# reesque/SfmFromScratch

Measured on AMD Instinct MI355X. Metric: images/sec detect+describe+match, 1080p, 1/2/4/8 MI355X, higher is better.
Workload: dtype f32; 1 GPU; BASELINE configs[1]: 32x 1080p per GPU, ScaleRotInvSIFT 4-level x2 octave pyramid, k=2500, fw 18, NNRatio 0.85 over consecutive pairs; frames_per_gpu=32, pairs_per_gpu=31, distinct_batches=2, parallelism=image-shard x1, batches_in_flight=2

## Files before the change

sfmfromscratch_amd/csrc/describe.hip:

```cpp
#include "kernels.h"

#include <stdlib.h>

namespace sfm {

SFM_DEV double pi_edge(int i, int num) {
  const double start = -3.141592653589793, stop = 3.141592653589793;
  if (i == num - 1) return stop;
  double step = (stop - start) / (double)(num - 1);
  return (double)i * step + start;
}

struct DescLayout {
  int ws, n, n4, pw, P;
  size_t off_keys, off_patch, off_ori, off_mag, off_sw, off_cw, off_cellw, off_wgh, total;
};

__host__ __device__ inline DescLayout desc_layout(int fw, int rotate) {
  DescLayout L;
  int h = fw / 2;
  L.ws = 2 * h;
  L.n = L.ws * L.ws;
  L.pw = L.ws + 2;
  int P = 1;
// ... 178 lines not shown
      for (int k = p; k >= 1; k >>= 1)
#pragma unroll
        for (int j = k % p; j + k < 16; j += 2 * k)
#pragma unroll
          for (int i = 0; i < k; ++i) {
            const int a = i + j, c = i + j + k;
            if (c < 16 && a / (2 * p) == c / (2 * p)) {
              const bool sw = cv[a] > cv[c] || (cv[a] == cv[c] && sl[a] > sl[c]);
              const double tv = cv[a];
              cv[a] = sw ? cv[c] : tv;
              cv[c] = sw ? tv : cv[c];
              const float tw = wt[a];
              wt[a] = sw ? wt[c] : tw;
              wt[c] = sw ? tw : wt[c];
              const int ts = sl[a];
              sl[a] = sw ? sl[c] : ts;
              sl[c] = sw ? ts : sl[c];
            }
          }
    float* cw = s_cellw + lane * 17;
    float acc = 0.0f;
    cw[0] = 0.0f;
#pragma unroll
    for (int m = 0; m < 16; ++m) {
      acc = acc + wt[m];
      cw[m + 1] = acc;
    }
    int idx[9];
#pragma unroll
    for (int eb = 0; eb < 9; ++eb) {
      const double e = pi_edge(eb, 9);
      int c = 0;
#pragma unroll
      for (int m = 0; m < 16; ++m) c += (eb < 8) ? (cv[m] < e ? 1 : 0) : (cv[m] <= e ? 1 : 0);
      idx[eb] = c;
    }
#pragma unroll
    for (int bb = 0; bb < 8; ++bb) s_wgh[lane * 8 + bb] = cw[idx[bb + 1]] - cw[idx[bb]];
  }
  __syncthreads();

  float w0 = s_wgh[lane], w1 = s_wgh[lane + 64];
  float a = w0 * w0;
  float c = w1 * w1;
  float s = a + c;
  for (int off = 32; off >= 1; off >>= 1) {
    float o = __shfl_down(s, off);
    s = s + o;
  }
  float nrm = sqrtf(__shfl(s, 0));
  int64_t off0 = 0;
  for (int l = 0; l < level; ++l) off0 += lc_all[(int64_t)l * B + b];
  const int64_t slot = (int64_t)b * out_cap + off0 + kpi;
  float v0 = w0, v1 = w1;
  if (nrm > 0.0f) {
    v0 = v0 / nrm;
    v1 = v1 / nrm;
  }
  out_desc[slot * 128 + lane] = sqrtf(v0);
  out_desc[slot * 128 + lane + 64] = sqrtf(v1);
  if (lane == 0) {
    if (out_conf) out_conf[slot] = kp.conf[ko];
    out_xy[slot * 2 + 0] = (int32_t)((double)x * scale);
    out_xy[slot * 2 + 1] = (int32_t)((double)y * scale);
  }
}

__global__ void k_finalize_counts(const int32_t* __restrict__ lc_all, int B, int L,
                                  int32_t* __restrict__ out_count) {
  int b = blockIdx.x * blockDim.x + threadIdx.x;
  if (b >= B) return;
  int32_t s = 0;
  for (int l = 0; l < L; ++l) s += lc_all[(int64_t)l * B + b];
  out_count[b] = s;
}

size_t describe_lds_bytes(int fw, int rotate) { return desc_layout(fw, rotate).total; }

void init_describe_attributes(size_t max_lds) {
  (void)hipFuncSetAttribute((const void*)k_describe, hipFuncAttributeMaxDynamicSharedMemorySize,
                            (int)max_lds);
}

bool launch_describe(const float* lvl, int B, int H, int W, int fw, int rotate, KpList kp,
                     int kcap, const int32_t* level_counts_all, int level, int L, double scale,
                     int32_t* out_xy, float* out_desc, float* out_conf, int64_t out_cap,
                     int32_t* out_count, const MatchOperands& mo, bool* operands_written, hipStream_t st) {
  if (operands_written) *operands_written = false;
  if (kcap <= 0) return false;
  static const bool one_per_wave = [] {
    const char* v = getenv("SFMFEAT_DESCRIBE");
    return v && v[0] == 'w';
  }();
  if (!one_per_wave && launch_describe_quad(lvl, B, H, W, fw, rotate, kp, kcap, level_counts_all, level,
                                            scale, out_xy, out_desc, out_conf, out_cap, out_count, L, mo, st)) {
    if (operands_written) *operands_written = mo.hi != nullptr;
    return out_count != nullptr;
  }
  size_t lds = describe_lds_bytes(fw, rotate);
  hipLaunchKernelGGL(k_describe, dim3(kcap, B), dim3(64), lds, st, lvl, H, W, fw, rotate, kp, kcap,
                     level_counts_all, level, B, scale, out_xy, out_desc, out_conf, out_cap);
  return false;
}

void launch_finalize_counts(const int32_t* level_counts_all, int B, int L, int32_t* out_count,
                            hipStream_t st) {
  hipLaunchKernelGGL(k_finalize_counts, dim3((B + 255) / 256), dim3(256), 0, st, level_counts_all, B, L,
                     out_count);
}

}
```

sfmfromscratch_amd/csrc/describe_q.hip:

```cpp
#include "kernels.h"

#include <stdlib.h>
#include <string.h>

#include <mutex>

namespace sfm {
namespace dq {

constexpr int cmax(int a, int b) { return a > b ? a : b; }
constexpr int pow2ceil(int v) { return v <= 1 ? 1 : 2 * pow2ceil((v + 1) / 2); }

template <int WS, int ROT>
struct Geo {
  static constexpr int N = WS * WS, PW = WS + 2, NP = PW * PW;
  static constexpr int P = cmax(pow2ceil(N), 16), E = P / 16;
  static constexpr int RN = (N + 15) / 16;
  static constexpr int A = (cmax(cmax(NP, N + 4), 16 * 17) + 3) & ~3;
  static constexpr int NQ = (N + 3) & ~3;
  static constexpr int OFF_M = A;
  static constexpr int OFF_K = OFF_M + NQ;
  static constexpr int OFF_R = OFF_K + NQ;
  static constexpr int OFF_I = OFF_R + (ROT ? (NQ / 2 + 3) & ~3 : 0);
  static constexpr int OFF_T = OFF_I + (ROT ? 40 : 0);
  static constexpr int G = OFF_T + 12;
};

SFM_DEV double pi_edge(int i, int num) {
  const double start = -3.141592653589793, stop = 3.141592653589793;
  if (i == num - 1) return stop;
  const double step = (stop - start) / (double)(num - 1);
  return (double)i * step + start;
}

SFM_DEV uint32_t edge_key(double e, double sh, bool strict) {
  uint32_t kc = fkey((float)(e + sh));
  auto pass = [&](uint32_t kk) {
    const double d = (double)fkey_inv(kk) - sh;
    return strict ? d > e : d >= e;
  };
  for (int it = 0; it < 64 && pass(kc); ++it) --kc;
  for (int it = 0; it < 64 && !pass(kc); ++it) ++kc;
  return kc;
}

__constant__ uint32_t c_ori[37];
__constant__ uint32_t c_cell[37][9];

template <int CTRL>
SFM_DEV uint32_t dpp(uint32_t v) {
  return (uint32_t)__builtin_amdgcn_update_dpp(0, (int)v, CTRL, 0xF, 0xF, true);
}
template <int X>
SFM_DEV uint32_t rxor(uint32_t v) {
  if constexpr (X == 1) return dpp<0xB1>(v);
  else if constexpr (X == 2) return dpp<0x4E>(v);
  else if constexpr (X == 3) return dpp<0x1B>(v);
  else if constexpr (X == 4) return dpp<0x1B>(dpp<0x141>(v));
  else if constexpr (X == 7) return dpp<0x141>(v);
  else if constexpr (X == 8) return dpp<0x128>(v);
  else {
    static_assert(X == 15, "row-local xor");
    return dpp<0x140>(v);
  }
}
template <int X>
SFM_DEV float rxorf(float v) { return __uint_as_float(rxor<X>(__float_as_uint(v))); }
template <int X>
SFM_DEV double rxord(double v) {
  const uint64_t u = __double_as_longlong(v);
  return __longlong_as_double((long long)(((uint64_t)rxor<X>((uint32_t)(u >> 32)) << 32) | rxor<X>((uint32_t)u)));
}

constexpr uint64_t kBias = 1ull << 52;
constexpr uint64_t kPad = kBias + (1ull << 41);
SFM_DEV double dkey(uint64_t payload) { return __longlong_as_double((long long)(kBias + payload)); }
SFM_DEV uint64_t dpayload(double k) { return (uint64_t)__double_as_longlong(k) - kBias; }

SFM_DEV void cas_up(double& a, double& b) {
  const double lo = __builtin_fmin(a, b), hi = __builtin_fmax(a, b);
  a = lo;
  b = hi;
}
SFM_DEV double keep_or_take(bool lower, double mine, double other) {
  const double lo = __builtin_fmin(mine, other), hi = __builtin_fmax(mine, other);
  return lower ? lo : hi;
}

template <int E, int S>
SFM_DEV void half_clean(double (&k)[E], int gl) {
  if constexpr (S >= 1) {
    if constexpr (S < E) {
#pragma unroll
      for (int r = 0; r < E; ++r)
        if ((r & S) == 0) cas_up(k[r], k[r + S]);
    } else {
      constexpr int X = S / E;
      const bool lower = (gl & X) == 0;
#pragma unroll
      for (int r = 0; r < E; ++r) k[r] = keep_or_take(lower, k[r], rxord<X>(k[r]));
    }
    half_clean<E, S / 2>(k, gl);
  }
}
template <int E, int SIZE>
SFM_DEV void merge_level(double (&k)[E], int gl) {
  if constexpr (SIZE <= 16 * E) {
    if constexpr (SIZE <= E) {
#pragma unroll
      for (int r = 0; r < E; ++r)
        if ((r & (SIZE / 2)) == 0) cas_up(k[r], k[r ^ (SIZE - 1)]);
    } else {
      constexpr int X = SIZE / E - 1;
      const bool lower = (gl & ((X + 1) >> 1)) == 0;
      if constexpr (E == 1) {
        k[0] = keep_or_take(lower, k[0], rxord<X>(k[0]));
      } else {
#pragma unroll
        for (int r = 0; r < E / 2; ++r) {
          const double oa = rxord<X>(k[E - 1 - r]);
          const double ob = rxord<X>(k[r]);
          k[r] = keep_or_take(lower, k[r], oa);
          k[E - 1 - r] = keep_or_take(lower, k[E - 1 - r], ob);
        }
      }
    }
    half_clean<E, SIZE / 4>(k, gl);
    merge_level<E, SIZE * 2>(k, gl);
  }
}

SFM_DEV void grad_at(const float* c, int pw, float& mag, float& ori) {
  const float a00 = c[-pw - 1], a01 = c[-pw], a02 = c[-pw + 1];
  const float a10 = c[-1], a12 = c[1];
  const float a20 = c[pw - 1], a21 = c[pw], a22 = c[pw + 1];
  float gx = 0.0f;
  gx = __builtin_fmaf(-1.0f, a00, gx);
  gx = __builtin_fmaf(1.0f, a02, gx);
  gx = __builtin_fmaf(-2.0f, a10, gx);
  gx = __builtin_fmaf(2.0f, a12, gx);
  gx = __builtin_fmaf(-1.0f, a20, gx);
  gx = __builtin_fmaf(1.0f, a22, gx);
  float gy = 0.0f;
  gy = __builtin_fmaf(-1.0f, a00, gy);
  gy = __builtin_fmaf(-2.0f, a01, gy);
  gy = __builtin_fmaf(-1.0f, a02, gy);
  gy = __builtin_fmaf(1.0f, a20, gy);
  gy = __builtin_fmaf(2.0f, a21, gy);
  gy = __builtin_fmaf(1.0f, a22, gy);
  const float sx = gx * gx;
  const float sy = gy * gy;
  const float s = sx + sy;
  mag = sqrtf(s);
  ori = svml_atan2f(gy, gx);
}

SFM_DEV void cas_up(uint32_t& a, uint32_t& b) {
  const uint32_t lo = min(a, b), hi = max(a, b);
  a = lo;
  b = hi;
}

template <typename T>
SFM_DEV void batcher16(T (&q)[16]) {
#pragma unroll
  for (int p = 1; p < 16; p <<= 1)
#pragma unroll
    for (int kk = p; kk >= 1; kk >>= 1)
#pragma unroll
      for (int j = kk % p; j + kk < 16; j += 2 * kk)
#pragma unroll
        for (int i = 0; i < kk; ++i) {
          const int a = i + j, c = i + j + kk;
          if (c < 16 && a / (2 * p) == c / (2 * p)) cas_up(q[a], q[c]);
        }
}

template <int WS, int ROT, int ABL = 0>
__global__ void __launch_bounds__(64) k_describe_q(const float* __restrict__ lvl, int H, int W, KpList kp,
                                                   int kcap, const int32_t* __restrict__ lc_all, int level,
                                                   int B, double scale, int32_t* __restrict__ out_xy,
                                                   float* __restrict__ out_desc, float* __restrict__ out_conf,
                                                   int64_t out_cap, int32_t* __restrict__ out_count, int L,
                                                   MatchOperands mo) {
  using C = Geo<WS, ROT>;
  constexpr int N = C::N, PW = C::PW, NP = C::NP, E = C::E, RN = C::RN, h = WS / 2;
  __shared__ __attribute__((aligned(16))) float s_all[4 * C::G];
  const int b = blockIdx.y;
  if (out_count != nullptr && blockIdx.x == 0 && threadIdx.x == 0) {
    int32_t s = 0;
    for (int l = 0; l < L; ++l) s += lc_all[(int64_t)l * B + b];
    out_count[b] = s;
  }
  const int nkb = (kcap + 3) / 4;
  if ((int)blockIdx.x >= nkb) {
    int32_t s = 0;
    for (int l = 0; l < L; ++l) s += lc_all[(int64_t)l * B + b];
    const int nt = ((int)gridDim.x - nkb) * 64;
    for (int64_t r = s + ((int)blockIdx.x - nkb) * 64 + threadIdx.x; r < mo.capP; r += nt) {
      const int64_t mr = (int64_t)b * mo.capP + r;
      uint4* hz = reinterpret_cast<uint4*>(mo.hi + mr * 128);
      uint4* lz = reinterpret_cast<uint4*>(mo.lo + mr * 128);
#pragma unroll
      for (int q = 0; q < 16; ++q) {
        hz[q] = make_uint4(0u, 0u, 0u, 0u);
        lz[q] = make_uint4(0u, 0u, 0u, 0u);
      }
      mo.norm2[mr] = INFINITY;
      mo.rnorm[mr] = 0.0f;
    }
    return;
  }
  const int count = kp.count[b];
  const int kbase = blockIdx.x * 4;
  if (kbase >= count) return;
  const int lane = threadIdx.x, g = lane >> 4, gl = lane & 15;
  const int kpi = kbase + g;
  const bool valid = kpi < count;
  const int64_t ko = (int64_t)b * kcap + (valid ? kpi : kbase);
  const int x = kp.x[ko], y = kp.y[ko];
  float* sA = s_all + g * C::G;
  float* sM = sA + C::OFF_M;
  uint32_t* sK = reinterpret_cast<uint32_t*>(sA + C::OFF_K);
  uint16_t* sR = reinterpret_cast<uint16_t*>(sA + C::OFF_R);
  int32_t* sI = reinterpret_cast<int32_t*>(sA + C::OFF_I);
  uint32_t* sT = reinterpret_cast<uint32_t*>(sA + C::OFF_T);

  const float* img = lvl + (int64_t)b * H * W;
#pragma unroll
  for (int it = 0; it < (NP + 15) / 16; ++it) {
    const int e0 = it * 16 + gl;
    const int e = e0 < NP ? e0 : NP - 1;
    const int pr = e / PW, pc = e - pr * PW;
    const int gy = y - h + pr, gx = x - h + pc;
    const bool in = gy >= 0 && gy < H && gx >= 0 && gx < W;
    const int cy = min(max(gy, 0), H - 1), cx = min(max(gx, 0), W - 1);
    const float v = (ABL & 64) ? (float)(cy + cx) : img[(int64_t)cy * W + cx];
    if (e0 < NP) sA[e] = in ? v : 0.0f;
  }
  __syncthreads();

  double k[E];
  bool tiny = false;
#pragma unroll
  for (int r = 0; r < E; ++r) k[r] = __longlong_as_double((long long)kPad);
#pragma unroll
  for (int r = 0; r < RN; ++r) {
    const int e0 = r * 16 + gl;
    const bool ok = (N % 16 == 0) || e0 < N;
    const int e = ok ? e0 : N - 1;
    const int i = e / WS, j = e - i * WS;
    float mag, ori;
    if constexpr ((ABL & 8) != 0) {
      mag = sA[(i + 1) * PW + (j + 1)];
      ori = sA[(i + 1) * PW + j] - 100.0f;
    } else {
      grad_at(sA + (i + 1) * PW + (j + 1), PW, mag, ori);
    }
    if (ok) {
      sM[e] = mag;
// ... 84 lines not shown
    }
    __syncthreads();
    float hb = -INFINITY;
    int bi = 64;
#pragma unroll
    for (int t = 0; t < 3; ++t) {
      const int j = gl + 16 * t;
      if (j < 36) {
        const float v = sA[3 + sI[j + 1]] - sA[3 + sI[j]];
        if (v > hb) { hb = v; bi = j; }
      }
    }
    {
      float ov; int oi;
      ov = rxorf<8>(hb); oi = (int)rxor<8>((uint32_t)bi);
      if (ov > hb || (ov == hb && oi < bi)) { hb = ov; bi = oi; }
      ov = rxorf<4>(hb); oi = (int)rxor<4>((uint32_t)bi);
      if (ov > hb || (ov == hb && oi < bi)) { hb = ov; bi = oi; }
      ov = rxorf<2>(hb); oi = (int)rxor<2>((uint32_t)bi);
      if (ov > hb || (ov == hb && oi < bi)) { hb = ov; bi = oi; }
      ov = rxorf<1>(hb); oi = (int)rxor<1>((uint32_t)bi);
      if (ov > hb || (ov == hb && oi < bi)) { hb = ov; bi = oi; }
    }
    dom = (pi_edge(bi, 37) + pi_edge(bi + 1, 37)) / 2.0;
    dom_bin = bi;
  }

  if (gl < 9) sT[gl] = (ABL & 32) ? 0x80000000u + (uint32_t)(dom * 1e6) * gl : c_cell[dom_bin][gl];
  __syncthreads();
  float hv[8];
  if constexpr ((ABL & 4) != 0) {
#pragma unroll
    for (int bb = 0; bb < 8; ++bb) hv[bb] = sM[gl * 8 + bb] + __uint_as_float(sT[bb & 7]);
  } else {
  const int r4 = gl >> 2, c4 = gl & 3;
  float wv[16];
  uint32_t hk[16];
  const bool grp_tiny = ROT && ((__ballot(tiny) >> (16 * g)) & 0xFFFFull) != 0;
  if (ROT && !grp_tiny) {
    uint32_t q[16];
#pragma unroll
    for (int t = 0; t < 16; ++t) {
      const int i = 4 * r4 + (t >> 2), j = 4 * c4 + (t & 3);
      const bool ok = i < WS && j < WS;
      q[t] = ok ? (uint32_t)sR[ok ? i * WS + j : 0] : 0xFFFFFFFFu;
    }
    batcher16(q);
#pragma unroll
    for (int m = 0; m < 16; ++m) {
      const bool ok = q[m] != 0xFFFFFFFFu;
      const uint32_t p = ok ? q[m] : 0u;
      wv[m] = ok ? sM[p] : 0.0f;
      hk[m] = ok ? sK[p] : 0xFFFFFFFFu;
    }
  } else {
    uint64_t q[16];
#pragma unroll
    for (int t = 0; t < 16; ++t) {
      const int i = 4 * r4 + (t >> 2), j = 4 * c4 + (t & 3);
      const bool ok = i < WS && j < WS;
      const int e = ok ? i * WS + j : 0;
      const uint32_t key = ROT ? sK[sR[e]] : fkey(__uint_as_float(sK[e]));
      q[t] = ok ? (((uint64_t)key << 32) | (uint32_t)t) : ~0ull;
    }
    if (!ROT) {
      double dq16[16];
#pragma unroll
      for (int t = 0; t < 16; ++t) dq16[t] = q[t] == ~0ull ? __longlong_as_double((long long)kPad)
                                                           : dkey(((q[t] >> 32) << 4) | (uint32_t)t);
      batcher16(dq16);
#pragma unroll
      for (int t = 0; t < 16; ++t) {
        const uint64_t pl = dpayload(dq16[t]);
        q[t] = pl >= (1ull << 36) ? ~0ull : (((pl >> 4) << 32) | (pl & 15u));
      }
    } else {
      double cv[16];
      int sl[16];
#pragma unroll
      for (int t = 0; t < 16; ++t) {
        cv[t] = q[t] == ~0ull ? INFINITY : (double)fkey_inv((uint32_t)(q[t] >> 32)) - dom;
        sl[t] = t;
      }
#pragma unroll
      for (int p = 1; p < 16; p <<= 1)
#pragma unroll
        for (int kk = p; kk >= 1; kk >>= 1)
#pragma unroll
          for (int j = kk % p; j + kk < 16; j += 2 * kk)
#pragma unroll
            for (int i = 0; i < kk; ++i) {
              const int a = i + j, c = i + j + kk;
              if (c < 16 && a / (2 * p) == c / (2 * p)) {
                const bool sw = cv[a] > cv[c] || (cv[a] == cv[c] && sl[a] > sl[c]);
                const double tv = cv[a];
                cv[a] = sw ? cv[c] : tv;
                cv[c] = sw ? tv : cv[c];
                const uint64_t tq = q[a];
                q[a] = sw ? q[c] : tq;
                q[c] = sw ? tq : q[c];
                const int ts = sl[a];
                sl[a] = sw ? sl[c] : ts;
                sl[c] = sw ? ts : sl[c];
              }
            }
    }
#pragma unroll
    for (int m = 0; m < 16; ++m) {
      const bool ok = q[m] != ~0ull;
      const int t = ok ? (int)(uint32_t)q[m] : 0;
      const int e = (4 * r4 + (t >> 2)) * WS + 4 * c4 + (t & 3);
      wv[m] = ok ? (ROT ? sM[sR[e]] : sM[e]) : 0.0f;
      hk[m] = ok ? (uint32_t)(q[m] >> 32) : 0xFFFFFFFFu;
    }
  }
  float* cc = sA + gl * 17;
  float acc = 0.0f;
  cc[0] = 0.0f;
#pragma unroll
  for (int m = 0; m < 16; ++m) {
    acc = acc + wv[m];
    cc[m + 1] = acc;
  }
  int bidx[9];
#pragma unroll
  for (int eb = 0; eb < 9; ++eb) {
    const uint32_t T = sT[eb];
    int c = 0;
#pragma unroll
    for (int m = 0; m < 16; ++m) c += hk[m] < T ? 1 : 0;
    bidx[eb] = c;
  }
#pragma unroll
  for (int bb = 0; bb < 8; ++bb) hv[bb] = cc[bidx[bb + 1]] - cc[bidx[bb]];

  }
  float tr[8];
#pragma unroll
  for (int t = 0; t < 8; ++t) {
    const float a = hv[t] * hv[t];
    tr[t] = a + rxorf<8>(a);
  }
#pragma unroll
  for (int t = 0; t < 8; ++t) tr[t] = tr[t] + rxorf<4>(tr[t]);
#pragma unroll
  for (int t = 0; t < 8; ++t) tr[t] = tr[t] + rxorf<2>(tr[t]);
#pragma unroll
  for (int t = 0; t < 8; ++t) tr[t] = tr[t] + rxorf<1>(tr[t]);
#pragma unroll
  for (int t = 0; t < 4; ++t) tr[t] = tr[t] + tr[t + 4];
  tr[0] = tr[0] + tr[2];
  tr[1] = tr[1] + tr[3];
  tr[0] = tr[0] + tr[1];
  const float nrm = sqrtf(__shfl(tr[0], g * 16));
  if (!valid) return;
  int64_t off0 = 0;
  for (int l = 0; l < level; ++l) off0 += lc_all[(int64_t)l * B + b];
  const int64_t slot = (int64_t)b * out_cap + off0 + kpi;
  float o[8];
#pragma unroll
  for (int t = 0; t < 8; ++t) o[t] = sqrtf(nrm > 0.0f ? hv[t] / nrm : hv[t]);
  float4* dst = reinterpret_cast<float4*>(out_desc + slot * 128 + gl * 8);
  dst[0] = make_float4(o[0], o[1], o[2], o[3]);
  dst[1] = make_float4(o[4], o[5], o[6], o[7]);
  if (mo.hi != nullptr) {
    const int64_t r = off0 + kpi, mr = (int64_t)b * mo.capP + r;
    typedef _Float16 h8 __attribute__((ext_vector_type(8)));
    h8 hh, ll;
    double s = 0.0;
#pragma unroll
    for (int t = 0; t < 8; ++t) {
      const float xs = o[t] * kMatchScale;
      const _Float16 hv16 = (_Float16)xs;
      const float rr = (xs - (float)hv16) * kMatchLoScale;
      hh[t] = hv16;
      ll[t] = (_Float16)rr;
      s += (double)o[t] * (double)o[t];
    }
    *reinterpret_cast<h8*>(mo.hi + mr * 128 + gl * 8) = hh;
    *reinterpret_cast<h8*>(mo.lo + mr * 128 + gl * 8) = ll;
    s += rxord<8>(s);
    s += rxord<4>(s);
    s += rxord<2>(s);
    s += rxord<1>(s);
    if (gl == 0) {
      const float n2 = (float)s, rn = (float)sqrt(s);
      mo.norm2[mr] = n2;
      mo.rnorm[mr] = rn;
      float2* pm = mo.pmax + (int64_t)b * (mo.capP / kPrepRows) + r / kPrepRows;
      atomicMax(reinterpret_cast<unsigned int*>(&pm->x), __float_as_uint(n2));
      atomicMax(reinterpret_cast<unsigned int*>(&pm->y), __float_as_uint(rn));
    }
  }
  if (gl == 0) {
    if (out_conf) out_conf[slot] = kp.conf[ko];
    out_xy[slot * 2 + 0] = (int32_t)((double)x * scale);
    out_xy[slot * 2 + 1] = (int32_t)((double)y * scale);
  }
}

}

namespace {
uint32_t fkey_h(float v) {
  uint32_t b;
  memcpy(&b, &v, 4);
  if (b == 0x80000000u) b = 0u;
  return (b & 0x80000000u) ? ~b : (b | 0x80000000u);
}
float fkey_inv_h(uint32_t k) {
  const uint32_t b = (k & 0x80000000u) ? (k & 0x7fffffffu) : ~k;
  float f;
  memcpy(&f, &b, 4);
  return f;
}
double pi_edge_h(int i, int num) {
  const double start = -3.141592653589793, stop = 3.141592653589793;
  if (i == num - 1) return stop;
  const double step = (stop - start) / (double)(num - 1);
  return (double)i * step + start;
}
uint32_t edge_key_h(double e, double sh, bool strict) {
  uint32_t kc = fkey_h((float)(e + sh));
  auto pass = [&](uint32_t kk) {
    const double d = (double)fkey_inv_h(kk) - sh;
    return strict ? d > e : d >= e;
  };
  for (int it = 0; it < 64 && pass(kc); ++it) --kc;
  for (int it = 0; it < 64 && !pass(kc); ++it) ++kc;
  return kc;
}
}

void init_describe_quad_tables() {
  static std::mutex mu;
  static bool done[256] = {};
  int dev = 0;
  if (hipGetDevice(&dev) != hipSuccess || dev < 0 || dev >= 256) return;
  std::lock_guard<std::mutex> lk(mu);
  if (done[dev]) return;
  uint32_t ori[37], cell[37][9];
  for (int j = 0; j < 37; ++j) ori[j] = edge_key_h(pi_edge_h(j, 37), 0.0, j == 36);
  for (int bi = 0; bi < 37; ++bi) {
    const double dom = bi < 36 ? (pi_edge_h(bi, 37) + pi_edge_h(bi + 1, 37)) / 2.0 : 0.0;
    for (int t = 0; t < 9; ++t) cell[bi][t] = edge_key_h(pi_edge_h(t, 9), dom, t == 8);
  }
  done[dev] = hipMemcpyToSymbol(HIP_SYMBOL(dq::c_ori), ori, sizeof(ori)) == hipSuccess &&
              hipMemcpyToSymbol(HIP_SYMBOL(dq::c_cell), cell, sizeof(cell)) == hipSuccess;
}

#define SFM_DQ_BODY(WS)                                                                              \
    if (rotate)                                                                                      \
      hipLaunchKernelGGL((dq::k_describe_q<WS, 1>), grid, dim3(64), 0, st, lvl, H, W, kp, kcap, lc,  \
                         level, B, scale, out_xy, out_desc, out_conf, out_cap, out_count, L, mo);        \
    else                                                                                             \
      hipLaunchKernelGGL((dq::k_describe_q<WS, 0>), grid, dim3(64), 0, st, lvl, H, W, kp, kcap, lc,  \
                         level, B, scale, out_xy, out_desc, out_conf, out_cap, out_count, L, mo);        \
    return true;
#define SFM_DQ_CASE(WS) \
  case WS:              \
    SFM_DQ_BODY(WS)

bool launch_describe_quad(const float* lvl, int B, int H, int W, int fw, int rotate, KpList kp, int kcap,
                          const int32_t* lc, int level, double scale, int32_t* out_xy, float* out_desc,
                          float* out_conf, int64_t out_cap, int32_t* out_count, int L, const MatchOperands& mo,
                          hipStream_t st) {
  constexpr int kPadBlocks = 8;
  const dim3 grid((kcap + 3) / 4 + (mo.hi != nullptr && out_count != nullptr ? kPadBlocks : 0), B);
  switch (2 * (fw / 2)) {
    SFM_DQ_CASE(2)
    SFM_DQ_CASE(4)
    SFM_DQ_CASE(6)
    SFM_DQ_CASE(8)
    SFM_DQ_CASE(10)
    SFM_DQ_CASE(12)
    SFM_DQ_CASE(14)
    SFM_DQ_CASE(16)
    case 18:
#ifdef SFM_ABLATIONS
      if (rotate) {
        static const int abl = [] {
          const char* v = SFM_ABLATION_ENV("SFMFEAT_DQ_ABL");
          return v ? atoi(v) : 0;
        }();
        switch (abl) {
#define SFM_DQ_ABL(A)                                                                                     \
  case A:                                                                                                \
    hipLaunchKernelGGL((dq::k_describe_q<18, 1, A>), grid, dim3(64), 0, st, lvl, H, W, kp, kcap, lc, level, \
                       B, scale, out_xy, out_desc, out_conf, out_cap, out_count, L, mo);                     \
    return true;
          SFM_DQ_ABL(1)
          SFM_DQ_ABL(2)
          SFM_DQ_ABL(4)
          SFM_DQ_ABL(8)
          SFM_DQ_ABL(7)
          SFM_DQ_ABL(16)
          SFM_DQ_ABL(32)
          SFM_DQ_ABL(64)
          SFM_DQ_ABL(55)
          SFM_DQ_ABL(127)
          default:
            break;
        }
      }
#endif
      SFM_DQ_BODY(18)
    SFM_DQ_CASE(20)
    SFM_DQ_CASE(22)
    default:
      return false;
  }
}

}
```

sfmfromscratch_amd/csrc/kernels.h:

```cpp
#pragma once

#include <hip/hip_runtime.h>
#include <stdint.h>

#include <vector>

#include "common.h"

namespace sfm {

#define SFM_NMS_MAX_HALF 15

constexpr int kHistBits = 12;
constexpr int kHistBins = 1 << kHistBits;
constexpr int kMedBits1 = 11;
constexpr int kMedBins1 = 1 << kMedBits1;
constexpr int kTopkLdsCap = 8192;
constexpr int kMaxMatchRows = 16384;
constexpr int kMatchCandCap = 256;
constexpr int kCounterStride = 32;
constexpr int kMatchUnitPairBits = 20;

constexpr float kMatchScale = 256.0f;
constexpr float kMatchLoScale = 2048.0f;
// ... 131 lines not shown

void ransac_sample_indices(int n, int iters, uint32_t seed, int32_t* out);
void launch_ransac(const int32_t* pts, const int32_t* npts, int nmax, int P, const int32_t* idx,
                   const int32_t* idx_off, int iters, double thr, double* Fs, int32_t* counts, int32_t* out_pts,
                   int32_t* out_n, int32_t* out_iter, hipStream_t st);

int build_resample_table(int in, int out, std::vector<int32_t>& tab);
bool ingest_rows_tables(const std::vector<int32_t>& tab_h, int ks_h, int W, int W2, int ks,
                        std::vector<int32_t>& colmap, std::vector<int32_t>& sets);
int ingest_rows_ks(int ks_h, int ks_v);
void launch_ingest_rgb(const uint8_t* rgb, uint8_t* tmp, float* gray, const int32_t* tab_h, int ks_h,
                       const int32_t* tab_v, int ks_v, const int32_t* colmap, const int32_t* sets, int nsets,
                       int B, int H, int W, int H2, int W2, hipStream_t st);
bool launch_down2x3(const float* src, int sh, int sw, float* d1, float* d2, float* d3, int B, hipStream_t st,
                    void* z0 = nullptr, size_t z0_bytes = 0, void* z1 = nullptr, size_t z1_bytes = 0);
void launch_resize(const float* src, int sh, int sw, float* dst, int dh, int dw, int B,
                   hipStream_t st);

void launch_harris(const float* lvl, float* R, uint32_t* hist, int B, int H, int W,
                   const float* d_gauss, int ks, float alpha, SelectScan scan, hipStream_t st);
constexpr int kHarrisMaxLevels = 4;
struct HarrisLevels {
  struct Level {
    const float* lvl;
    float* R;
    uint32_t* hist;
    int H, W, tiles_x, ntiles, wg0, nwg;
    SelectScan scan;
    float* down[3];
  } l[kHarrisMaxLevels];
  int n;
  int prio;
  int stagger;
  unsigned long long* span;
};
void launch_harris_levels(const HarrisLevels& g, int B, const float* d_gauss, int ks, float alpha,
                          hipStream_t st);
constexpr int kHarrisPairOff = 256;
size_t harris_taps_floats(int ks);
void harris_taps_build(const float* g, int ks, float* out);

int64_t match_stamps_copy(uint64_t* out, int64_t cap);
size_t match_units_words(int P, int max_rows);
float time_harris_ablation(int abl, const float* lvl, float* R, uint32_t* hist, int B, int H, int W,
                           const float* gk, float alpha, int iters, uint64_t* stamps = nullptr,
                           int64_t stamps_cap = 0);

void launch_select_scan(const uint32_t* hist, MedianState* state, unsigned long long* list_count, int B,
                        int H, int W, int64_t vmin, int force_exact, hipStream_t st);
void launch_median_exact(const float* R, MedianState* state, uint32_t* list, unsigned long long* list_count,
                         int B, int H, int W, hipStream_t st);

void launch_nms(const float* R, const MedianState* state, uint64_t* cand,
                unsigned long long* cand_count, int B, int H, int W, int ksize, int mode, hipStream_t st,
                int force_tile = 0);

void init_topk_attributes();
void init_describe_attributes(size_t max_lds);
void init_describe_quad_tables();
size_t describe_lds_bytes(int fw, int rotate);
void launch_select(const float* R, uint64_t* cand, const unsigned long long* cand_count, uint32_t* medlist,
                   uint64_t* scratch, KpList kp, int kcap, int k, int B, int H, int W, int ksize, int half_window,
                   MedianState* state, hipStream_t st);
constexpr int kSelectMaxLevels = 4;
struct SelectLevels {
  struct Level {
    const float* R;
    uint64_t* cand;
    const unsigned long long* cand_count;
    uint32_t* medlist;
    uint64_t* scratch;
    KpList kp;
    MedianState* state;
    int H, W, hw;
  } l[kSelectMaxLevels];
  int n;
};
void launch_select_levels(const SelectLevels& g, int kcap, int k, int B, int ksize, hipStream_t st);

bool launch_describe_quad(const float* lvl, int B, int H, int W, int fw, int rotate, KpList kp, int kcap,
                          const int32_t* level_counts_all, int level, double scale, int32_t* out_xy,
                          float* out_desc, float* out_conf, int64_t out_cap, int32_t* out_count, int L,
                          const MatchOperands& mo, hipStream_t st);
bool launch_describe(const float* lvl, int B, int H, int W, int fw, int rotate, KpList kp,
                     int kcap, const int32_t* level_counts_all, int level, int L, double scale,
                     int32_t* out_xy, float* out_desc, float* out_conf, int64_t out_cap,
                     int32_t* out_count, const MatchOperands& mo, bool* operands_written, hipStream_t st);
void launch_finalize_counts(const int32_t* level_counts_all, int B, int L, int32_t* out_count,
                            hipStream_t st);

struct RowBest {
  int32_t col;
  float nndr;
};
void launch_transpose_desc(const float* desc, const int32_t* count, int nimg, int64_t cap,
                           int64_t capP, float* descT, hipStream_t st);
void launch_match_rows(const float* descT, const int32_t* count, int64_t capP, const int32_t* pairs,
                       int P, float ratio, RowBest* rows, int max_rows, hipStream_t st);
void launch_match_compact(const RowBest* rows, const int32_t* count, const int32_t* pairs, int P,
                          int max_rows, int64_t cap, int32_t* matches, float* conf, int32_t* nmatch,
                          int* reset_counter, hipStream_t st);
void init_match_attributes(int max_rows);
size_t match_pmax_bytes(int64_t capP);
void launch_match_prep(const float* desc, const int32_t* count, int nimg, int64_t cap, int64_t capP,
                       _Float16* hi, _Float16* lo, float* norm2, float* rnorm, void* pmax, hipStream_t st);
void launch_match_mfma(const float* desc, const int32_t* count, int64_t cap, int64_t capP,
                       const _Float16* hi, const _Float16* lo, const float* norm2, const float* rnorm,
                       const void* pmax, const int32_t* pairs, int P, float ratio,
                       RowBest* rows, int max_rows, uint32_t* cand, int32_t* cand_n, float* cand_thr,
                       int* ovf_count, int2* ovf_list, int32_t* units, hipStream_t st);

}
```

sfmfromscratch_amd/csrc/sfmfeat_api.hip:

```cpp
#include <math.h>
#include <stdio.h>
#include <stdlib.h>
#include <string.h>

#include <algorithm>
#include <atomic>
#include <string>
#include <thread>
#include <vector>

#include "../../include/sfmfeat.h"
#include "kernels.h"

using namespace sfm;

namespace {

struct DevBuf {
  void* p = nullptr;
  size_t bytes = 0;
};

struct Level {
  int h, w, fw;
// ... 395 lines not shown
    return SFM_OK;
  };
  for (int l0 = 0; l0 < L;) {
    int l1 = l0 + 1;
    if (group_from > 0 && l0 >= group_from) l1 = std::min(L, l0 + kHarrisMaxLevels);
    {
      StageScope sc(c, SFM_PROF_HARRIS, st);
      HarrisLevels g{};
      g.n = l1 - l0;
      for (int l = l0; l < l1; ++l) {
        const LevelBufs& e = lb[l];
        HarrisLevels::Level& q = g.l[l - l0];
        q.lvl = lvl[l];
        q.R = e.R;
        q.hist = as<uint32_t>(c->d_hist) + (size_t)l * B * kMedBins1;
        q.H = lv[l].h;
        q.W = lv[l].w;
        q.scan = SelectScan{e.med, medcnt + e.co, donecnt + e.co, vmin, e.exact ? 1 : 0};
        q.down[0] = q.down[1] = q.down[2] = nullptr;
        if (pyr_fused && l == 0) {
          q.down[0] = const_cast<float*>(lvl[1]);
          q.down[1] = const_cast<float*>(lvl[2]);
          q.down[2] = const_cast<float*>(lvl[3]);
        }
      }
      if (c->span_cap > 0) {
        if (c->span_n < c->span_cap) {
          g.span = as<unsigned long long>(c->d_spans) + 2 * c->span_n++;
          c->span_level.push_back(l0);
        } else {
          ++c->span_dropped;
        }
      }
      if (!(l0 > 0 && (skip & 16))) launch_harris_levels(g, B, as<float>(c->d_gauss), c->p.gaussian_size, alpha, st);
    }
    if (pyr_fused && l0 == 0 && L > 4) {
      StageScope sc(c, SFM_PROF_PYRAMID, st);
      pyramid_from(4);
    }
    if (gate_level >= l0 && gate_level < l1 && (rc = release_gate())) return rc;
    for (int l = l0; l < l1; ++l) {
      const LevelBufs& e = lb[l];
      if (!e.exact) {
        StageScope sc(c, SFM_PROF_NMS, st);
        launch_nms(e.R, e.med, e.cand, candcnt + e.co, B, lv[l].h, lv[l].w, c->p.ksize, 0, st);
      }
      if (l < L_aux) {
        static const bool sel_caller = [] {
          const char* e = SFM_DIAG_ENV("SFMFEAT_SELECT_CALLER");
          return e && atoi(e) == 1;
        }();
        if (sel_caller) select_level(l, st);
        HIPCHK(c, hipEventRecord(c->ev[l], st));
        HIPCHK(c, hipStreamWaitEvent(ax, c->ev[l], 0));
        if (!sel_caller) select_level(l, ax);
        if (l == L_aux - 1) HIPCHK(c, hipEventRecord(c->ev[L + 2], ax));
        describe_level(l, ax);
      }
    }
    l0 = l1;
  }
  if ((rc = release_gate())) return rc;
  static const bool merge_select = [] {
    const char* e = SFM_DIAG_ENV("SFMFEAT_SELECT_MERGE");
    return !(e && atoi(e) == 0);
  }();
  if (merge_select && L - L_aux > 1 && L - L_aux <= kSelectMaxLevels) {
    StageScope sc(c, SFM_PROF_TOPK, st);
    SelectLevels g{};
    g.n = L - L_aux;
    int64_t so = L_aux > 0 ? (int64_t)B * H * W : 0;
    for (int l = L_aux; l < L; ++l) {
      const LevelBufs& e = lb[l];
      g.l[l - L_aux] = SelectLevels::Level{e.R, e.cand, candcnt + e.co, as<uint32_t>(c->d_medlist) + so,
                                           as<uint64_t>(c->d_scratch) + so, e.kp, e.med, lv[l].h, lv[l].w,
                                           lv[l].fw / 2};
      so += (int64_t)B * lv[l].h * lv[l].w;
    }
    if (!(skip & 1)) launch_select_levels(g, std::max(c->kcap, 1), c->kcap, B, c->p.ksize, st);
  } else {
    for (int l = L_aux; l < L; ++l) select_level(l, st);
  }
  if (L_aux > 0 && L > L_aux) HIPCHK(c, hipStreamWaitEvent(st, c->ev[L + 2], 0));
  for (int l = L_aux; l < L; ++l) describe_level(l, st);
  if (L_aux > 0) {
    HIPCHK(c, hipEventRecord(c->ev[L + 1], ax));
    HIPCHK(c, hipStreamWaitEvent(st, c->ev[L + 1], 0));
  }
  if (!counted) launch_finalize_counts(as<int32_t>(c->d_lc), B, L, count, st);
  HIPCHK(c, hipGetLastError());
  if (fused_ok && counted) {
    c->fp_desc = desc;
    c->fp_count = count;
    c->fp_cap = cap;
    c->fp_B = B;
  }
  return SFM_OK;
}

int match_prep_range(sfm_ctx* c, const float* desc, const int32_t* count, int nimg, int64_t cap, int lo, int n,
                     hipStream_t st) {
  if (cap < 1 || cap > kMaxMatchRows)
    return set_err(c, SFM_EINVAL, "match capacity must be in [1, 16384]");
  if (lo < 0 || n < 0 || lo + n > nimg) return set_err(c, SFM_EINVAL, "prep slot range outside the table");
  int rc;
  const float* d0 = desc + (int64_t)lo * cap * 128;
  c->prep_desc = desc;
  c->prep_count = count;
  c->prep_nimg = nimg;
  c->prep_cap = cap;
  if (c->match_direct) {
    const int64_t capP = (cap + 63) / 64 * 64;
    if ((rc = ensure(c, c->m_descT, (size_t)nimg * 128 * capP * 4))) return rc;
    if (n == 0) return SFM_OK;
    StageScope sc(c, SFM_PROF_MATCH_PREP, st);
    launch_transpose_desc(d0, count + lo, n, cap, capP, as<float>(c->m_descT) + (int64_t)lo * 128 * capP, st);
  } else {
    const int64_t capP = (cap + 127) / 128 * 128;
    if ((rc = match_operands_reserve(c, nimg, capP))) return rc;
    if (n == 0) return SFM_OK;
    StageScope sc(c, SFM_PROF_MATCH_PREP, st);
    const int64_t o = (int64_t)lo * capP;
    launch_match_prep(d0, count + lo, n, cap, capP, as<_Float16>(c->m_hi) + o * 128, as<_Float16>(c->m_lo) + o * 128,
                      as<float>(c->m_norm2) + o, as<float>(c->m_rnorm) + o,
                      as<char>(c->m_imgmax) + (size_t)lo * match_pmax_bytes(capP), st);
  }
  HIPCHK(c, hipGetLastError());
  return SFM_OK;
}

int match_impl(sfm_ctx* c, const float* desc, const int32_t* count, int nimg, int64_t cap,
               const int32_t* pairs, int P, float ratio, int32_t* matches, float* conf,
               int32_t* nmatch, hipStream_t st, bool prep = true) {
  if (P <= 0) return SFM_OK;
  if (cap < 1 || cap > kMaxMatchRows)
    return set_err(c, SFM_EINVAL, "match capacity must be in [1, 16384]");
  int rc;
  if (prep) {
    int lo = 0;
    if (!c->match_direct && c->fp_desc == desc && c->fp_count == count && c->fp_cap == cap && c->fp_B <= nimg &&
        match_operands_fit(c, nimg, (cap + 127) / 128 * 128))
      lo = c->fp_B;
    if ((rc = match_prep_range(c, desc, count, nimg, cap, lo, nimg - lo, st))) return rc;
  } else {
    if (c->prep_desc != desc || c->prep_count != count || c->prep_nimg != nimg || c->prep_cap != cap)
      return set_err(c, SFM_ESTATE, "sfm_match_pairs_prepped_dev: this table was not the last one prepped "
                                    "(sfm_match_prep_dev) on this context");
  }
  const size_t budget = c->match_budget;
  const size_t per_pair = (size_t)cap * (sizeof(RowBest) + sizeof(int2) + (c->match_direct ? 0 : kMatchCandCap * 4 + 8));
  const int Pmax = (int)std::max<size_t>(
      1, std::min<size_t>(std::min<size_t>((size_t)P, budget / per_pair), (size_t)1 << kMatchUnitPairBits));
  if ((rc = ensure(c, c->m_rows, (size_t)Pmax * cap * sizeof(RowBest)))) return rc;
  if ((rc = ensure(c, c->m_ovf, (size_t)Pmax * cap * sizeof(int2)))) return rc;
  if (c->m_ovfc.bytes == 0) {
    if ((rc = ensure(c, c->m_ovfc, 16))) return rc;
    HIPCHK(c, hipMemsetAsync(c->m_ovfc.p, 0, 16, st));
  }
  if (!c->match_direct) {
    if ((rc = ensure(c, c->m_cand, (size_t)Pmax * cap * kMatchCandCap * 4))) return rc;
    if ((rc = ensure(c, c->m_candn, (size_t)Pmax * cap * 4))) return rc;
    if ((rc = ensure(c, c->m_candt, (size_t)Pmax * cap * 4))) return rc;
    if ((rc = ensure(c, c->m_units, match_units_words(Pmax, (int)cap) * 4))) return rc;
  }
  for (int p0 = 0; p0 < P; p0 += Pmax, ++c->match_calls) {
    const int Pn = std::min(Pmax, P - p0);
    const int32_t* pr = pairs + 2 * (int64_t)p0;
// ... 707 lines not shown
```

Measured before the change: 42900 images/sec.

## Merge small-window describe levels into one packed multi-level kernel launch

Adds a describe kernel that packs 16 keypoints per 64-thread block, four lanes per keypoint, for window sizes 2 and 4. It also handles all trailing small-window pyramid levels in one launch instead of one launch per level. The new kernel uses a reduced-width bitonic merge, binary-search histogram binning and fused count/operand padding. This cuts per-level launch overhead and the underused lanes of the one-keypoint-per-quad kernel, at the cost of more complex code and a fallback path when the levels are not contiguous.

```diff
diff --git a/sfmfromscratch_amd/csrc/describe.hip b/sfmfromscratch_amd/csrc/describe.hip
--- a/sfmfromscratch_amd/csrc/describe.hip
+++ b/sfmfromscratch_amd/csrc/describe.hip
@@ -284,17 +284,34 @@
                             (int)max_lds);
 }
 
+static bool describe_one_per_wave() {
+  static const bool one_per_wave = [] {
+    const char* v = getenv("SFMFEAT_DESCRIBE");
+    return v && v[0] == 'w';
+  }();
+  return one_per_wave;
+}
+
+bool launch_describe_levels(const DescribeLevels& g, int B, int rotate, int kcap, const int32_t* level_counts_all,
+                            int32_t* out_xy, float* out_desc, float* out_conf, int64_t out_cap,
+                            int32_t* out_count, int L, const MatchOperands& mo, bool* operands_written,
+                            hipStream_t st) {
+  if (operands_written) *operands_written = false;
+  if (describe_one_per_wave() ||
+      !launch_describe_small(g, B, rotate, kcap, level_counts_all, out_xy, out_desc, out_conf, out_cap, out_count,
+                             L, mo, st))
+    return false;
+  if (operands_written) *operands_written = mo.hi != nullptr;
+  return true;
+}
+
 bool launch_describe(const float* lvl, int B, int H, int W, int fw, int rotate, KpList kp,
                      int kcap, const int32_t* level_counts_all, int level, int L, double scale,
                      int32_t* out_xy, float* out_desc, float* out_conf, int64_t out_cap,
                      int32_t* out_count, const MatchOperands& mo, bool* operands_written, hipStream_t st) {
   if (operands_written) *operands_written = false;
   if (kcap <= 0) return false;
-  static const bool one_per_wave = [] {
-    const char* v = getenv("SFMFEAT_DESCRIBE");
-    return v && v[0] == 'w';
-  }();
-  if (!one_per_wave && launch_describe_quad(lvl, B, H, W, fw, rotate, kp, kcap, level_counts_all, level,
+  if (!describe_one_per_wave() && launch_describe_quad(lvl, B, H, W, fw, rotate, kp, kcap, level_counts_all, level,
                                             scale, out_xy, out_desc, out_conf, out_cap, out_count, L, mo, st)) {
     if (operands_written) *operands_written = mo.hi != nullptr;
     return out_count != nullptr;
diff --git a/sfmfromscratch_amd/csrc/describe_q.hip b/sfmfromscratch_amd/csrc/describe_q.hip
--- a/sfmfromscratch_amd/csrc/describe_q.hip
+++ b/sfmfromscratch_amd/csrc/describe_q.hip
@@ -87,7 +87,7 @@
   return lower ? lo : hi;
 }
 
-template <int E, int S>
+template <int E, int S, int LPK = 16>
 SFM_DEV void half_clean(double (&k)[E], int gl) {
   if constexpr (S >= 1) {
     if constexpr (S < E) {
@@ -100,12 +100,12 @@
 #pragma unroll
       for (int r = 0; r < E; ++r) k[r] = keep_or_take(lower, k[r], rxord<X>(k[r]));
     }
-    half_clean<E, S / 2>(k, gl);
-  }
-}
-template <int E, int SIZE>
+    half_clean<E, S / 2, LPK>(k, gl);
+  }
+}
+template <int E, int SIZE, int LPK = 16>
 SFM_DEV void merge_level(double (&k)[E], int gl) {
-  if constexpr (SIZE <= 16 * E) {
+  if constexpr (SIZE <= LPK * E) {
     if constexpr (SIZE <= E) {
 #pragma unroll
       for (int r = 0; r < E; ++r)
@@ -125,8 +125,8 @@
         }
       }
     }
-    half_clean<E, SIZE / 4>(k, gl);
-    merge_level<E, SIZE * 2>(k, gl);
+    half_clean<E, SIZE / 4, LPK>(k, gl);
+    merge_level<E, SIZE * 2, LPK>(k, gl);
   }
 }
 
@@ -176,6 +176,26 @@
         }
 }
 
+#define SFM_BATCHER16_REL(cv, q, sl)                                                   \
+  _Pragma("unroll") for (int p = 1; p < 16; p <<= 1)                                   \
+  _Pragma("unroll") for (int kk = p; kk >= 1; kk >>= 1)                                \
+  _Pragma("unroll") for (int j = kk % p; j + kk < 16; j += 2 * kk)                     \
+  _Pragma("unroll") for (int i = 0; i < kk; ++i) {                                     \
+    const int a = i + j, c = i + j + kk;                                               \
+    if (c < 16 && a / (2 * p) == c / (2 * p)) {                                        \
+      const bool sw = cv[a] > cv[c] || (cv[a] == cv[c] && sl[a] > sl[c]);              \
+      const double tv = cv[a];                                                         \
+      cv[a] = sw ? cv[c] : tv;                                                         \
+      cv[c] = sw ? tv : cv[c];                                                         \
+      const uint64_t tq = q[a];                                                        \
+      q[a] = sw ? q[c] : tq;                                                           \
+      q[c] = sw ? tq : q[c];                                                           \
+      const int ts = sl[a];                                                            \
+      sl[a] = sw ? sl[c] : ts;                                                         \
+      sl[c] = sw ? ts : sl[c];                                                         \
+    }                                                                                  \
+  }
+
 template <int WS, int ROT, int ABL = 0>
 __global__ void __launch_bounds__(64) k_describe_q(const float* __restrict__ lvl, int H, int W, KpList kp,
                                                    int kcap, const int32_t* __restrict__ lc_all, int level,
@@ -426,28 +446,7 @@
         cv[t] = q[t] == ~0ull ? INFINITY : (double)fkey_inv((uint32_t)(q[t] >> 32)) - dom;
         sl[t] = t;
       }
-#pragma unroll
-      for (int p = 1; p < 16; p <<= 1)
-#pragma unroll
-        for (int kk = p; kk >= 1; kk >>= 1)
-#pragma unroll
-          for (int j = kk % p; j + kk < 16; j += 2 * kk)
-#pragma unroll
-            for (int i = 0; i < kk; ++i) {
-              const int a = i + j, c = i + j + kk;
-              if (c < 16 && a / (2 * p) == c / (2 * p)) {
-                const bool sw = cv[a] > cv[c] || (cv[a] == cv[c] && sl[a] > sl[c]);
-                const double tv = cv[a];
-                cv[a] = sw ? cv[c] : tv;
-                cv[c] = sw ? tv : cv[c];
-                const uint64_t tq = q[a];
-                q[a] = sw ? q[c] : tq;
-                q[c] = sw ? tq : q[c];
-                const int ts = sl[a];
-                sl[a] = sw ? sl[c] : ts;
-                sl[c] = sw ? ts : sl[c];
-              }
-            }
+      SFM_BATCHER16_REL(cv, q, sl)
     }
 #pragma unroll
     for (int m = 0; m < 16; ++m) {
@@ -543,6 +542,286 @@
   }
 }
 
+struct Q4 {
+  static constexpr int OFF_M = 40;
+  static constexpr int OFF_KE = 56;
+  static constexpr int OFF_K = 72;
+  static constexpr int OFF_C = 88;
+  static constexpr int OFF_B = 108;
+  static constexpr int G = 124;
+};
+constexpr int kQ4Pack = 16;
+
+template <int N>
+SFM_DEV int lower_count(const uint32_t* sK, uint32_t T) {
+  int lo = 0;
+  constexpr int S0 = pow2ceil(N + 1) / 2;
+#pragma unroll
+  for (int it = 0; (S0 >> it) >= 1; ++it) {
+    const int q = lo + (S0 >> it);
+    const uint32_t v = sK[(q <= N ? q : N) - 1];
+    if (q <= N && v < T) lo = q;
+  }
+  return lo;
+}
+
+template <int WS, int ROT>
+SFM_DEV void describe_q4_body(float* s_all, const DescribeLevels::Level& lv, int kbase, int b, int kcap,
+                              const int32_t* __restrict__ lc_all, int B, int32_t* __restrict__ out_xy,
+                              float* __restrict__ out_desc, float* __restrict__ out_conf, int64_t out_cap,
+                              const MatchOperands& mo) {
+  constexpr int N = WS * WS, PW = WS + 2, NP = PW * PW, E = N / 4, h = WS / 2;
+  static_assert(NP <= Q4::OFF_M && N <= 16 && NP % 4 == 0, "one cell");
+  const int H = lv.H, W = lv.W;
+  const int count = lv.kp.count[b];
+  if (kbase >= count) return;
+  const int lane = threadIdx.x, g = lane >> 2, ql = lane & 3;
+  const int kpi = kbase + g;
+  const bool valid = kpi < count;
+  const int64_t ko = (int64_t)b * kcap + (valid ? kpi : kbase);
+  const int x = lv.kp.x[ko], y = lv.kp.y[ko];
+  float* sA = s_all + g * Q4::G;
+  int32_t* sI = reinterpret_cast<int32_t*>(sA);
+  float* sM = sA + Q4::OFF_M;
+  uint32_t* sKe = reinterpret_cast<uint32_t*>(sA + Q4::OFF_KE);
+  uint32_t* sK = reinterpret_cast<uint32_t*>(sA + Q4::OFF_K);
+  float* sC = sA + Q4::OFF_C;
+  int32_t* sB = reinterpret_cast<int32_t*>(sA + Q4::OFF_B);
+
+  const float* img = lv.lvl + (int64_t)b * H * W;
+#pragma unroll
+  for (int it = 0; it < NP / 4; ++it) {
+    const int e = it * 4 + ql;
+    const int pr = e / PW, pc = e - pr * PW;
+    const int gy = y - h + pr, gx = x - h + pc;
+    const bool in = gy >= 0 && gy < H && gx >= 0 && gx < W;
+    const int cy = min(max(gy, 0), H - 1), cx = min(max(gx, 0), W - 1);
+    const float v = img[(int64_t)cy * W + cx];
+    sA[e] = in ? v : 0.0f;
+  }
+  __syncthreads();
+
+  double k[E];
+  bool tiny = false;
+#pragma unroll
+  for (int r = 0; r < E; ++r) {
+    const int e = r * 4 + ql;
+    const int i = e / WS, j = e - i * WS;
+    float mag, ori;
+    grad_at(sA + (i + 1) * PW + (j + 1), PW, mag, ori);
+    const uint32_t fk = fkey(ori);
+    sM[e] = mag;
+    if (ROT) sKe[e] = fk;
+    k[r] = dkey(((uint64_t)fk << 9) | (uint32_t)e);
+    tiny |= ROT && ori != 0.0f && fabsf(ori) < 0x1p-25f;
+  }
+  __syncthreads();
+
+  merge_level<E, 2, 4>(k, ql);
+  float w[E], cw[E];
+  uint32_t kf[E];
+#pragma unroll
+  for (int r = 0; r < E; ++r) {
+    const uint64_t pl = dpayload(k[r]);
+    kf[r] = (uint32_t)(pl >> 9);
+    w[r] = sM[(uint32_t)(pl & 511u)];
+    cw[r] = 0.0f;
+  }
+  float carry = 0.0f;
+#pragma unroll
+  for (int s = 0; s < 4; ++s) {
+    if (ql == s) {
+      float acc = carry;
+#pragma unroll
+      for (int r = 0; r < E; ++r) {
+        acc = acc + w[r];
+        cw[r] = acc;
+      }
+    }
+    const float nxt = __uint_as_float(dpp<0x90>(__float_as_uint(cw[E - 1])));
+    if (ql == s + 1) carry = nxt;
+  }
+#pragma unroll
+  for (int r = 0; r < E; ++r) {
+    sK[ql * E + r] = kf[r];
+    sC[1 + ql * E + r] = cw[r];
+  }
+  if (ql == 0) sC[0] = 0.0f;
+  __syncthreads();
+
+  double dom = 0.0;
+  int dom_bin = 36;
+  if constexpr (ROT) {
+#pragma unroll
+    for (int t = 0; t < 10; ++t) {
+      const int j = ql + 4 * t;
+      if (j <= 36) sI[j] = lower_count<N>(sK, c_ori[j]);
+    }
+    __syncthreads();
+    float hb = -INFINITY;
+    int bi = 64;
+#pragma unroll
+    for (int t = 0; t < 9; ++t) {
+      const int j = ql + 4 * t;
+      const float v = sC[sI[j + 1]] - sC[sI[j]];
+      if (v > hb) { hb = v; bi = j; }
+    }
+    {
+      float ov; int oi;
+      ov = rxorf<2>(hb); oi = (int)rxor<2>((uint32_t)bi);
+      if (ov > hb || (ov == hb && oi < bi)) { hb = ov; bi = oi; }
+      ov = rxorf<1>(hb); oi = (int)rxor<1>((uint32_t)bi);
+      if (ov > hb || (ov == hb && oi < bi)) { hb = ov; bi = oi; }
+    }
+    dom = (pi_edge(bi, 37) + pi_edge(bi + 1, 37)) / 2.0;
+    dom_bin = bi;
+  }
+
+#pragma unroll
+  for (int t = 0; t < 3; ++t) {
+    const int eb = ql + 4 * t;
+    if (eb < 9) sB[eb] = lower_count<N>(sK, c_cell[dom_bin][eb]);
+  }
+  float wt[16];
+  const bool grp_tiny = ROT && ((__ballot(tiny) >> (4 * g)) & 0xFull) != 0;
+  if (grp_tiny) {
+    uint64_t q[16];
+    double cv[16];
+    int sl[16];
+#pragma unroll
+    for (int t = 0; t < 16; ++t) {
+      const int i = t >> 2, j = t & 3;
+      const bool ok = i < WS && j < WS;
+      const int e = ok ? i * WS + j : 0;
+      q[t] = ok ? (uint64_t)__float_as_uint(sM[e]) : 0ull;
+      cv[t] = ok ? (double)fkey_inv(sKe[e]) - dom : INFINITY;
+      sl[t] = t;
+    }
+    SFM_BATCHER16_REL(cv, q, sl)
+#pragma unroll
+    for (int m = 0; m < 16; ++m) wt[m] = __uint_as_float((uint32_t)q[m]);
+  }
+  __syncthreads();
+  if (grp_tiny) {
+    float acc = 0.0f;
+#pragma unroll
+    for (int m = 0; m < N; ++m) {
+      acc = acc + wt[m];
+      if (ql == 0) sC[m + 1] = acc;
+    }
+  }
+  __syncthreads();
+  float hv[8];
+  {
+    float cb[9];
+#pragma unroll
+    for (int eb = 0; eb < 9; ++eb) cb[eb] = sC[sB[eb]];
+#pragma unroll
+    for (int bb = 0; bb < 8; ++bb) hv[bb] = cb[bb + 1] - cb[bb];
+  }
+  float tr[8];
+#pragma unroll
+  for (int t = 0; t < 8; ++t) tr[t] = hv[t] * hv[t];
+#pragma unroll
+  for (int t = 0; t < 4; ++t) tr[t] = tr[t] + tr[t + 4];
+  tr[0] = tr[0] + tr[2];
+  tr[1] = tr[1] + tr[3];
+  tr[0] = tr[0] + tr[1];
+  const float nrm = sqrtf(tr[0]);
+  if (!valid) return;
+  int64_t off0 = 0;
+  for (int l = 0; l < lv.level; ++l) off0 += lc_all[(int64_t)l * B + b];
+  const int64_t slot = (int64_t)b * out_cap + off0 + kpi;
+  float o[8];
+#pragma unroll
+  for (int t = 0; t < 8; ++t) o[t] = sqrtf(nrm > 0.0f ? hv[t] / nrm : hv[t]);
+  float4* dst = reinterpret_cast<float4*>(out_desc + slot * 128);
+  const float4 z4 = make_float4(0.0f, 0.0f, 0.0f, 0.0f);
+  dst[ql] = ql == 0 ? make_float4(o[0], o[1], o[2], o[3]) : ql == 1 ? make_float4(o[4], o[5], o[6], o[7]) : z4;
+#pragma unroll
+  for (int i = 1; i < 8; ++i) dst[ql + 4 * i] = z4;
+  if (mo.hi != nullptr) {
+    const int64_t r = off0 + kpi, mr = (int64_t)b * mo.capP + r;
+    typedef _Float16 h8 __attribute__((ext_vector_type(8)));
+    h8 hh, ll, zz;
+    double s = 0.0;
+#pragma unroll
+    for (int t = 0; t < 8; ++t) {
+      const float xs = o[t] * kMatchScale;
+      const _Float16 hv16 = (_Float16)xs;
+      const float rr = (xs - (float)hv16) * kMatchLoScale;
+      hh[t] = hv16;
+      ll[t] = (_Float16)rr;
+      zz[t] = (_Float16)0.0f;
+      s += (double)o[t] * (double)o[t];
+    }
+    h8* hrow = reinterpret_cast<h8*>(mo.hi + mr * 128);
+    h8* lrow = reinterpret_cast<h8*>(mo.lo + mr * 128);
+    hrow[ql] = ql == 0 ? hh : zz;
+    lrow[ql] = ql == 0 ? ll : zz;
+#pragma unroll
+    for (int i = 1; i < 4; ++i) {
+      hrow[ql + 4 * i] = zz;
+      lrow[ql + 4 * i] = zz;
+    }
+    if (ql == 0) {
+      const float n2 = (float)s, rn = (float)sqrt(s);
+      mo.norm2[mr] = n2;
+      mo.rnorm[mr] = rn;
+      float2* pm = mo.pmax + (int64_t)b * (mo.capP / kPrepRows) + r / kPrepRows;
+      atomicMax(reinterpret_cast<unsigned int*>(&pm->x), __float_as_uint(n2));
+      atomicMax(reinterpret_cast<unsigned int*>(&pm->y), __float_as_uint(rn));
+    }
+  }
+  if (ql == 0) {
+    if (out_conf) out_conf[slot] = lv.kp.conf[ko];
+    out_xy[slot * 2 + 0] = (int32_t)((double)x * lv.scale);
+    out_xy[slot * 2 + 1] = (int32_t)((double)y * lv.scale);
+  }
+}
+
+template <int ROT>
+__global__ void __launch_bounds__(64) k_describe_q4(DescribeLevels g, int kcap, const int32_t* __restrict__ lc_all,
+                                                    int B, int32_t* __restrict__ out_xy,
+                                                    float* __restrict__ out_desc, float* __restrict__ out_conf,
+                                                    int64_t out_cap, int32_t* __restrict__ out_count, int L,
+                                                    MatchOperands mo) {
+  __shared__ __attribute__((aligned(16))) float s_all[kQ4Pack * Q4::G];
+  const int b = blockIdx.y;
+  if (out_count != nullptr && blockIdx.x == 0 && threadIdx.x == 0) {
+    int32_t s = 0;
+    for (int l = 0; l < L; ++l) s += lc_all[(int64_t)l * B + b];
+    out_count[b] = s;
+  }
+  if ((int)blockIdx.x >= g.nblk) {
+    int32_t s = 0;
+    for (int l = 0; l < L; ++l) s += lc_all[(int64_t)l * B + b];
+    const int nt = ((int)gridDim.x - g.nblk) * 64;
+    for (int64_t r = s + ((int)blockIdx.x - g.nblk) * 64 + threadIdx.x; r < mo.capP; r += nt) {
+      const int64_t mr = (int64_t)b * mo.capP + r;
+      uint4* hz = reinterpret_cast<uint4*>(mo.hi + mr * 128);
+      uint4* lz = reinterpret_cast<uint4*>(mo.lo + mr * 128);
+#pragma unroll
+      for (int q = 0; q < 16; ++q) {
+        hz[q] = make_uint4(0u, 0u, 0u, 0u);
+        lz[q] = make_uint4(0u, 0u, 0u, 0u);
+      }
+      mo.norm2[mr] = INFINITY;
+      mo.rnorm[mr] = 0.0f;
+    }
+    return;
+  }
+  int li = 0;
+  for (int i = 1; i < g.n; ++i)
+    if ((int)blockIdx.x >= g.l[i].blk0) li = i;
+  const DescribeLevels::Level& lv = g.l[li];
+  const int kbase = ((int)blockIdx.x - lv.blk0) * kQ4Pack;
+  if (lv.ws == 2)
+    describe_q4_body<2, ROT>(s_all, lv, kbase, b, kcap, lc_all, B, out_xy, out_desc, out_conf, out_cap, mo);
+  else
+    describe_q4_body<4, ROT>(s_all, lv, kbase, b, kcap, lc_all, B, out_xy, out_desc, out_conf, out_cap, mo);
+}
+
 }
 
 namespace {
@@ -593,7 +872,28 @@
               hipMemcpyToSymbol(HIP_SYMBOL(dq::c_cell), cell, sizeof(cell)) == hipSuccess;
 }
 
-#define SFM_DQ_BODY(WS)                                                                              \
+bool launch_describe_small(DescribeLevels g, int B, int rotate, int kcap, const int32_t* lc, int32_t* out_xy,
+                           float* out_desc, float* out_conf, int64_t out_cap, int32_t* out_count, int L,
+                           const MatchOperands& mo, hipStream_t st) {
+  if (g.n < 1 || g.n > kSelectMaxLevels || kcap <= 0 || B < 1) return false;
+  const int per_level = (kcap + dq::kQ4Pack - 1) / dq::kQ4Pack;
+  for (int i = 0; i < g.n; ++i) {
+    if (g.l[i].ws != 2 && g.l[i].ws != 4) return false;
+    g.l[i].blk0 = i * per_level;
+  }
+  g.nblk = g.n * per_level;
+  constexpr int kPadBlocks = 8;
+  const dim3 grid(g.nblk + (mo.hi != nullptr && out_count != nullptr ? kPadBlocks : 0), B);
+  if (rotate)
+    hipLaunchKernelGGL((dq::k_describe_q4<1>), grid, dim3(64), 0, st, g, kcap, lc, B, out_xy, out_desc, out_conf,
+                       out_cap, out_count, L, mo);
+  else
+    hipLaunchKernelGGL((dq::k_describe_q4<0>), grid, dim3(64), 0, st, g, kcap, lc, B, out_xy, out_desc, out_conf,
+                       out_cap, out_count, L, mo);
+  return true;
+}
+
+#define SFM_DQ_BODY(WS)                                                                             \
     if (rotate)                                                                                      \
       hipLaunchKernelGGL((dq::k_describe_q<WS, 1>), grid, dim3(64), 0, st, lvl, H, W, kp, kcap, lc,  \
                          level, B, scale, out_xy, out_desc, out_conf, out_cap, out_count, L, mo);        \
@@ -612,8 +912,14 @@
   constexpr int kPadBlocks = 8;
   const dim3 grid((kcap + 3) / 4 + (mo.hi != nullptr && out_count != nullptr ? kPadBlocks : 0), B);
   switch (2 * (fw / 2)) {
-    SFM_DQ_CASE(2)
-    SFM_DQ_CASE(4)
+    case 2:
+    case 4: {
+      DescribeLevels g{};
+      g.n = 1;
+      g.l[0] = DescribeLevels::Level{lvl, kp, scale, H, W, 2 * (fw / 2), level, 0};
+      return launch_describe_small(g, B, rotate, kcap, lc, out_xy, out_desc, out_conf, out_cap, out_count, L, mo,
+                                   st);
+    }
     SFM_DQ_CASE(6)
     SFM_DQ_CASE(8)
     SFM_DQ_CASE(10)
diff --git a/sfmfromscratch_amd/csrc/kernels.h b/sfmfromscratch_amd/csrc/kernels.h
--- a/sfmfromscratch_amd/csrc/kernels.h
+++ b/sfmfromscratch_amd/csrc/kernels.h
@@ -237,6 +237,22 @@
                           const int32_t* level_counts_all, int level, double scale, int32_t* out_xy,
                           float* out_desc, float* out_conf, int64_t out_cap, int32_t* out_count, int L,
                           const MatchOperands& mo, hipStream_t st);
+struct DescribeLevels {
+  struct Level {
+    const float* lvl;
+    KpList kp;
+    double scale;
+    int H, W, ws, level, blk0;
+  } l[kSelectMaxLevels];
+  int n, nblk;
+};
+bool launch_describe_small(DescribeLevels g, int B, int rotate, int kcap, const int32_t* level_counts_all,
+                           int32_t* out_xy, float* out_desc, float* out_conf, int64_t out_cap,
+                           int32_t* out_count, int L, const MatchOperands& mo, hipStream_t st);
+bool launch_describe_levels(const DescribeLevels& g, int B, int rotate, int kcap, const int32_t* level_counts_all,
+                            int32_t* out_xy, float* out_desc, float* out_conf, int64_t out_cap,
+                            int32_t* out_count, int L, const MatchOperands& mo, bool* operands_written,
+                            hipStream_t st);
 bool launch_describe(const float* lvl, int B, int H, int W, int fw, int rotate, KpList kp,
                      int kcap, const int32_t* level_counts_all, int level, int L, double scale,
                      int32_t* out_xy, float* out_desc, float* out_conf, int64_t out_cap,
diff --git a/sfmfromscratch_amd/csrc/sfmfeat_api.hip b/sfmfromscratch_amd/csrc/sfmfeat_api.hip
--- a/sfmfromscratch_amd/csrc/sfmfeat_api.hip
+++ b/sfmfromscratch_amd/csrc/sfmfeat_api.hip
@@ -501,7 +501,29 @@
     for (int l = L_aux; l < L; ++l) select_level(l, st);
   }
   if (L_aux > 0 && L > L_aux) HIPCHK(c, hipStreamWaitEvent(st, c->ev[L + 2], 0));
-  for (int l = L_aux; l < L; ++l) describe_level(l, st);
+  int l_small = L;
+  while (l_small > L_aux && L - l_small < kSelectMaxLevels &&
+         (lv[l_small - 1].fw / 2 == 1 || lv[l_small - 1].fw / 2 == 2))
+    --l_small;
+  for (int l = L_aux; l < l_small; ++l) describe_level(l, st);
+  bool merged = false;
+  if (L - l_small > 1 && !(skip & 2)) {
+    StageScope sc(c, SFM_PROF_DESCRIBE, st);
+    DescribeLevels g{};
+    g.n = L - l_small;
+    for (int l = l_small; l < L; ++l)
+      g.l[l - l_small] =
+          DescribeLevels::Level{lvl[l], lb[l].kp, lv[l].scale, lv[l].h, lv[l].w, 2 * (lv[l].fw / 2), l, 0};
+    bool ow = false;
+    merged = launch_describe_levels(g, B, rotate, c->kcap, as<int32_t>(c->d_lc), xy, desc, conf, cap, count, L, mo,
+                                    &ow, st);
+    if (merged) {
+      counted = true;
+      fused_ok = fused_ok && ow;
+    }
+  }
+  if (!merged)
+    for (int l = l_small; l < L; ++l) describe_level(l, st);
   if (L_aux > 0) {
     HIPCHK(c, hipEventRecord(c->ev[L + 1], ax));
     HIPCHK(c, hipStreamWaitEvent(st, c->ev[L + 1], 0));
```

Result: no change. 43160 images/sec, median of 6 (+0.6%).
